# retab-dev/k-LLMs

Measured on NVIDIA H100. Metric: consensus records/sec at n=16 (1M x 32-field); achieved HBM GB/s vs peak, higher is better.
Workload: dtype i32 codes / f64 values

## Files before the change

### k_llms_b200/csrc/kc_jsongpu.cu

```cuda
#include <cuda_runtime.h>

#include <algorithm>
#include <atomic>
#include <chrono>
#include <cstdio>
#include <cstdlib>
#include <cstring>
#include <mutex>
#include <string>
#include <thread>
#include <type_traits>
#include <vector>

#include <cub/device/device_scan.cuh>
#include <nvtx3/nvToolsExt.h>

#include "../../include/kllms_b200.h"
#include "kc_internal.h"
#include "kc_jsongpu.cuh"

namespace {

using kc::js::Chunk;
using kc::js::Tok;
// ... 57 lines not shown
    }
    template <typename T>
    T *as() const { return static_cast<T *>(p); }
};

enum Stage { RECORDS, SLOTS, UNION, SCRATCH, CSR, OFF };
struct Units {
    size_t R, B, T = 0, P = 0, S = 0;
};
template <class Alloc>
int chunk_arrays(const Alloc &alloc, Chunk &ch, Stage stage, const Units &u, size_t keep, bool vrec) {
    const size_t n = (size_t)ch.n;
    int k = 0;
    auto a = [&](Stage st, auto *&ptr, size_t count, size_t per, size_t plus, int fill, bool on_device) {
        const int i = k++;
        return st == stage ? alloc(i, ptr, count * per + plus, keep * per, fill, on_device) : KC_OK;
    };
    R_(a(RECORDS, ch.fcount, u.R, 1, 1, 0, true));
    R_(a(RECORDS, ch.slot, u.R, 1, 1, 0, false));
    R_(a(RECORDS, ch.status, u.R, 1, 0, 0, false));
    R_(a(RECORDS, ch.nest, u.R, 1, 0, 0, false));
    R_(a(RECORDS, ch.pend, u.R, 1, 0, 0, false));
    R_(a(RECORDS, ch.plist, u.R, 1, 1, 0xFF, false));
    R_(a(ch.lists ? RECORDS : OFF, ch.lst, u.R, 1, 0, 0, false));
    R_(a(RECORDS, ch.vbase, u.R, 1, 0, 0, false));
    R_(a(RECORDS, ch.xbase, u.R, 1, 0, 0, false));
    R_(a(RECORDS, ch.mcount, u.R, 1, 1, 0, true));
    R_(a(RECORDS, ch.scount, u.R, 1, 1, 0, true));
    R_(a(RECORDS, ch.ccount, u.R, 1, 1, 0, true));
    R_(a(RECORDS, ch.len_c, u.R, 1, 1, 0, true));
    R_(a(RECORDS, ch.len_l, u.R, 1, 1, 0, true));
    R_(a(SLOTS, ch.toks, u.T, n, 1, 0, false));
    R_(a(SLOTS, ch.fdesc, u.T, 1, 1, 0, false));
    R_(a(SLOTS, ch.gpos, u.T, 1, 1, 0, false));
    R_(a(SLOTS, ch.piece_c, u.T, 1, 1, 0, false));
    R_(a(SLOTS, ch.piece_l, u.T, 1, 1, 0, false));
    R_(a(SLOTS, ch.vcells, u.T, n, 16, 0xFF, true));
    R_(a(SLOTS, ch.xcells, u.T, n, 2, 0, true));
    R_(a(vrec ? SLOTS : OFF, ch.vrec, u.T, 1, 1, 0xFF, false));
    R_(a(UNION, ch.ucand, u.P, n, 0, 0, false));
    R_(a(UNION, ch.ubase, u.P, 1, 0, 0, false));
    R_(a(UNION, ch.usize, u.P, 1, 0, 0, false));
    R_(a(SCRATCH, ch.utok, u.S, 1, 0, 0, false));
    R_(a(SCRATCH, ch.unode, u.S, 1, 0, 0, false));
    R_(a(SCRATCH, ch.umap, u.S, 1, 0, 0xFF, false));
    R_(a(CSR, ch.mchars, u.B, 1, 16, 0, false));
    R_(a(CSR, ch.mstr_off, u.T, n, 2, 0, false));
    R_(a(CSR, ch.mgrp_off, u.T, 1, 2, 0, false));
    return KC_OK;
}

void set_flags(Chunk &ch, uint32_t flags, uint8_t lists, int32_t aligned0) {
    ch.xmedoid = (flags & KC_JSON_NUMERIC_MEDOID) != 0;
    ch.key_union = (flags & KC_JSON_KEY_UNION) != 0;
    ch.unicode = (flags & KC_JSON_UNICODE) != 0;
    ch.lists = lists;
    ch.aligned0 = aligned0;
}

struct Worker {
    int device = -1;
    cudaStream_t stream = nullptr;
    cudaEvent_t ev[7] = {};
    DBuf text, off, counters, win, vmeta, xvalue, xmeta, out_c, out_l, scan_tmp, midx, mavg, seq, vweight;
    std::vector<DBuf> arrays;
    PBuf h_small;
// ... 635 lines not shown
    if (!res) return;
    release_blob(res->blob);
    delete res;
}


struct kc_debug_jsongpu {
    std::vector<int64_t> off;
    std::vector<uint8_t> text;
    int32_t n = 0;
    int64_t R = 0;
    std::vector<std::vector<uint8_t>> arrays;
    unsigned long long counters[6] = {0, 0, 0, 0, 0, 0};
    std::vector<uint8_t> out_c, out_l;
    int64_t R_out = 0;
    std::vector<int64_t> src;
    std::vector<int64_t> spliced_c, spliced_l;
    std::vector<uint8_t> spliced_out_c, spliced_out_l;
    Chunk ch{};
};

int kc_debug_jsongpu_plan(const char *h_text, const int64_t *h_off, int64_t n_records, int32_t n, kc_debug_jsongpu **out) {
    return kc_debug_jsongpu_plan_flags(h_text, h_off, n_records, n, 0u, out);
}

namespace {

void plan_twin(kc_debug_jsongpu *h, const char *h_text, const int64_t *h_off, int64_t R, int32_t n, uint32_t flags, uint8_t lists, int32_t aligned0) {
    h->R = R;
    h->R_out = R;
    h->n = n;
    h->off.assign(h_off, h_off + R * n + 1);
    h->text.assign((const uint8_t *)h_text + h_off[0], (const uint8_t *)h_text + h_off[R * n]);
    Chunk &ch = h->ch;
    ch.text = h->text.data();
    ch.off = h->off.data();
    ch.R = (int32_t)R;
    ch.n = n;
    ch.counters = h->counters;
    set_flags(ch, flags, lists, aligned0);
    auto host = [&](int k, auto *&ptr, size_t len, size_t, int fill, bool) -> int {
        using E = std::remove_reference_t<decltype(*ptr)>;
        if (h->arrays.size() <= (size_t)k) h->arrays.resize((size_t)k + 1);
        h->arrays[(size_t)k].resize(len * sizeof(E), (uint8_t)fill);
        ptr = reinterpret_cast<E *>(h->arrays[(size_t)k].data());
        return KC_OK;
    };
    Units u{(size_t)R, h->text.size()};
    chunk_arrays(host, ch, RECORDS, u, 0, true);
    for (int32_t r = 0; r < R; ++r) kc::js::count_record(ch, r);
    for (int64_t r = 0; r < R; ++r) ch.slot[r + 1] = ch.slot[r] + ch.fcount[r];
    u.T = ch.slot[R];
    chunk_arrays(host, ch, SLOTS, u, 0, true);
    const kc::js::HostTeam team{team_size(n)};
    for (int32_t r = 0; r < R; ++r) kc::js::plan_step(ch, r, team);
    if ((u.P = h->counters[3])) {
        const int32_t P = (int32_t)u.P;
        chunk_arrays(host, ch, UNION, u, 0, true);
        ch.uslot = (uint32_t)u.T;
        for (int32_t p = 0; p < P; ++p) kc::js::union_count_step(ch, p, team);
        u.S = std::max<size_t>(h->counters[4], 1);
        chunk_arrays(host, ch, SCRATCH, u, 0, true);
        for (int32_t p = 0; p < P; ++p) kc::js::union_build_step(ch, p, team);
        const size_t keep = u.T;
        u.T += h->counters[5];
        chunk_arrays(host, ch, SLOTS, u, keep, true);
        for (int32_t p = 0; p < P; ++p) kc::js::union_plan_step(ch, p, team);
    }
    for (uint32_t *cnt : {ch.mcount, ch.scount, ch.ccount}) exclusive_scan(cnt, u.R + 1);
    chunk_arrays(host, ch, CSR, u, 0, true);
    for (int32_t r = 0; r < R; ++r) kc::js::medoid_step(ch, r, team);
}

}

int kc_debug_jsongpu_plan_flags(const char *h_text, const int64_t *h_off, int64_t n_records, int32_t n, uint32_t flags,
                                kc_debug_jsongpu **out) {
    if (!h_text || !h_off || !out || n < 2 || n > KC_MAX_CANDIDATES || n_records < 0) return KC_EINVAL;
    const int64_t R = n_records;
    kc_debug_jsongpu *h = new kc_debug_jsongpu;
    const bool lists = (flags & KC_JSON_LISTS) != 0;
// ... 48 lines not shown
int kc_debug_jsongpu_set_medoid(kc_debug_jsongpu *h, const int32_t *medoid_idx, const double *medoid_avg) {
    if (!h) return KC_EINVAL;
    h->ch.midx = medoid_idx;
    h->ch.mavg = medoid_avg;
    return KC_OK;
}

int kc_debug_jsongpu_set_numeric_medoid(kc_debug_jsongpu *h, const int32_t *best, const double *best_avg) {
    if (!h) return KC_EINVAL;
    h->ch.xbest = best;
    h->ch.xavg = best_avg;
    return KC_OK;
}

int kc_debug_jsongpu_inputs(const kc_debug_jsongpu *h, const int8_t **vote_cells, int64_t *n_vote_groups, const double **num_cells,
                            int64_t *n_num_groups, const uint8_t **status) {
    if (!h) return KC_EINVAL;
    if (vote_cells) *vote_cells = h->ch.vcells;
    if (n_vote_groups) *n_vote_groups = (int64_t)h->counters[0];
    if (num_cells) *num_cells = h->ch.xcells;
    if (n_num_groups) *n_num_groups = (int64_t)h->counters[1];
    if (status) *status = h->ch.status;
    return KC_OK;
}

int kc_debug_jsongpu_emit(kc_debug_jsongpu *h, const uint32_t *vote_meta, const double *num_value, const uint32_t *num_meta,
                          const char **content, const int64_t **content_off, const char **likelihoods, const int64_t **likelihoods_off) {
    return kc_debug_jsongpu_emit_weighted(h, vote_meta, nullptr, num_value, num_meta, content, content_off, likelihoods, likelihoods_off);
}

int kc_debug_jsongpu_group_records(const kc_debug_jsongpu *h, const int32_t **group_record) {
    if (!h) return KC_EINVAL;
    if (group_record) *group_record = h->ch.vrec;
    return KC_OK;
}

int kc_debug_jsongpu_emit_weighted(kc_debug_jsongpu *h, const uint32_t *vote_meta, const float *vote_weight, const double *num_value,
                                   const uint32_t *num_meta, const char **content, const int64_t **content_off, const char **likelihoods,
                                   const int64_t **likelihoods_off) {
    if (!h) return KC_EINVAL;
    Chunk &ch = h->ch;
    ch.vmeta = vote_meta;
    ch.vweight = vote_weight;
    ch.xvalue = num_value;
    ch.xmeta = num_meta;
    const int64_t R = h->R;
    const kc::js::HostTeam team{team_size(h->n)};
    for (int32_t r = 0; r < R; ++r) kc::js::len_step(ch, r, team);
    exclusive_scan(ch.len_c, (size_t)R + 1);
    exclusive_scan(ch.len_l, (size_t)R + 1);
    const int64_t ac = ch.len_c[R], al = ch.len_l[R];
    h->out_c.assign((size_t)std::max<int64_t>(ac, 1), 0);
    h->out_l.assign((size_t)std::max<int64_t>(al, 1), 0);
    ch.out_c = h->out_c.data();
    ch.out_l = h->out_l.data();
    for (int32_t r = 0; r < R; ++r) kc::js::write_step(ch, r, team);
    if (h->R_out < R) {
        const int64_t Ro = h->R_out;
        std::vector<int64_t> from((size_t)Ro);
        for (int64_t r = 0; r < Ro; ++r) from[(size_t)r] = r;
        for (int64_t i = 0; i < R - Ro; ++i) {
            from[(size_t)h->src[(size_t)i]] = Ro + i;
            ch.status[h->src[(size_t)i]] = ch.status[Ro + i];
        }
        auto splice = [&](const int64_t *o, const std::vector<uint8_t> &blob, std::vector<int64_t> &so, std::vector<uint8_t> &sb) {
            so.assign((size_t)Ro + 1, 0);
// ... 249 lines not shown
```

### k_llms_b200/csrc/kc_jsongpu.cuh

```cuda
#pragma once

#include "kc_jsoncore.cuh"

namespace kc {
namespace js {

constexpr int32_t kMaxFields = 1024;

constexpr uint8_t D_UNION = 0xFF;
constexpr uint8_t D_LIST = 0xFE;

struct UNode {
    uint32_t kstart;
    uint16_t klen;
    uint8_t depth;
    uint8_t obj;
    uint8_t scalar;
    int32_t parent, child, last, next;
    int32_t lastc;
    uint32_t row, close;
};

KC_HD inline uint32_t fdesc_pack(uint32_t kind, uint32_t last, uint32_t rank, uint32_t gidx) { return kind | (last << 4) | (rank << 5) | (gidx << 16); }
KC_HD inline uint32_t fdesc_kind(uint32_t d) { return d & 15u; }
KC_HD inline uint32_t fdesc_last(uint32_t d) { return (d >> 4) & 1u; }
KC_HD inline uint32_t fdesc_rank(uint32_t d) { return (d >> 5) & 0x7FFu; }
KC_HD inline uint32_t fdesc_gidx(uint32_t d) { return d >> 16; }

struct Chunk {
    const uint8_t *text;
    const int64_t *off;
    int32_t R, n;
    uint32_t *fcount;
    uint8_t *nest;
    uint32_t *gpos;
    uint32_t *slot;
    uint8_t *status;
    Tok *toks;
    uint32_t *fdesc;
    uint32_t *vbase, *xbase;
    unsigned long long *counters;
    int8_t *vcells;
    double *xcells;
    uint32_t *mcount, *scount, *ccount;
    uint8_t *mchars;
    int32_t *mstr_off, *mgrp_off;
    const int32_t *midx;
    const double *mavg;
    int32_t *vrec;
    const float *vweight;
    const uint32_t *vmeta;
    const double *xvalue;
    const uint32_t *xmeta;
    bool xmedoid;
    const int32_t *xbest;
    const double *xavg;
    uint32_t *piece_c, *piece_l;
    int64_t *len_c, *len_l;
    uint8_t *out_c, *out_l;
    uint8_t *pend;
    int32_t *plist;
    uint32_t *ucand;
    uint32_t *ubase;
    uint32_t *usize;
    Tok *utok;
    UNode *unode;
    int32_t *umap;
    uint32_t uslot;
    bool key_union;
    uint8_t *lst;
    uint8_t lists;
    int32_t aligned0;
// ... 48 lines not shown
            decline(ch, r, D_LIST);
        } else if (f == -D_TOO_MANY_FIELDS || (f >= 0 && f != F)) {
            differ(ch, r, D_KEYS_DIFFER);
        } else if (f < 0) {
            decline(ch, r, -f);
        }
    }
}

KC_HD inline void settle_listed(const Chunk &ch, int32_t r) {
    int32_t why = D_LIST;
    for (int32_t c = 0; c < ch.n && why == D_LIST; ++c) {
        int64_t b, len;
        const int64_t base0 = ch.off[0];
        b = ch.off[(int64_t)r * ch.n + c] - base0;
        len = ch.off[(int64_t)r * ch.n + c + 1] - base0 - b;
        int32_t f = -D_TOO_LONG;
        if (len < ((int64_t)1 << 31)) f = scan_object(ch.text + b, (uint32_t)len, 0, nullptr, 0, kMaxFields, nullptr, true, nullptr, ch.unicode);
        if (f < 0) why = -f;
    }
    decline(ch, r, why);
}

KC_HD inline void sibling_range(const Tok *rt, int32_t n, int32_t F, int32_t j, uint32_t d, bool flat, int32_t &lo, int32_t &hi) {
    lo = 0;
    hi = F;
    if (flat) return;
    lo = j;
    while (lo > 0 && tok_depth(rt[(int64_t)(lo - 1) * n]) >= d) --lo;
    hi = j + 1;
    while (hi < F && tok_depth(rt[(int64_t)hi * n]) >= d) ++hi;
}

KC_HD inline void type_phase(const Chunk &ch, int32_t r, int32_t lane, int32_t team) {
    if (load_status(ch, r)) return;
    const int32_t F = (int32_t)ch.fcount[r], n = ch.n;
    const bool flat = ch.nest[r] == 0;
    const Tok *rt = ch.toks + (int64_t)ch.slot[r] * n;
    for (int32_t j = lane; j < F; j += team) {
        const Tok *row = rt + (int64_t)j * n;
        const uint32_t k0 = row[0].kind, d = tok_depth(row[0]);
        int32_t ref = j;
        if (is_close(k0)) {
            for (int32_t c = 1; c < n; ++c)
                if (row[c].kind != k0 || tok_depth(row[c]) != d) {
                    differ(ch, r, D_KEYS_DIFFER);
                    return;
                }
            ref = j - 1;
            while (ref > 0 && tok_depth(rt[(int64_t)ref * n]) != d) --ref;
        }
        const uint8_t *key = ch.text + rt[(int64_t)ref * n].kstart;
        const uint32_t klen = rt[(int64_t)ref * n].klen;
        const uint8_t elem = rt[(int64_t)ref * n].flags & TOK_ELEM;
        if (!is_close(k0)) {
            for (int32_t c = 1; c < n; ++c) {
                if ((row[c].kind == K_OPEN) != (k0 == K_OPEN) || (row[c].kind == K_LOPEN) != (k0 == K_LOPEN) || is_close(row[c].kind)) {
                    differ(ch, r, D_NESTED);
                    return;
                }
                if (tok_depth(row[c]) != d || (row[c].flags & TOK_ELEM) != elem || row[c].klen != klen ||
                    key_compare(ch.text + row[c].kstart, klen, key, klen) != 0) {
                    differ(ch, r, D_KEYS_DIFFER);
                    return;
                }
            }
            if (!elem && (contains(key, klen, "reasoning___", 12) || contains(key, klen, "source___", 9) ||
                          (F == 1 && klen == 4 && key_compare(key, 4, (const uint8_t *)"text", 4) == 0))) {
                decline(ch, r, D_SPECIAL_KEY);
                return;
            }
        }
        int32_t lo, hi;
        sibling_range(rt, n, F, ref, d, flat, lo, hi);
        uint32_t rank = 0, after = 0;
        for (int32_t i = lo; i < hi; ++i) {
            const Tok &o = rt[(int64_t)i * n];
            if (i == ref || (!flat && (tok_depth(o) != d || is_close(o.kind)))) continue;
            if (elem) {
                rank += i < ref ? 1u : 0u;
                after += i > ref ? 1u : 0u;
                continue;
            }
            const int cmp = key_compare(ch.text + o.kstart, o.klen, key, klen);
            if (cmp == 0) {
                decline(ch, r, D_DUP_KEY);
                return;
            }
            rank += cmp < 0 ? 1u : 0u;
            after += cmp > 0 ? 1u : 0u;
        }
        const uint32_t last = after == 0 ? 1u : 0u;
        if (is_open(k0) || is_close(k0)) {
            const uint32_t kind = k0 == K_OPEN ? F_OPEN : (k0 == K_CLOSE ? F_CLOSE : (k0 == K_LOPEN ? F_LOPEN : F_LCLOSE));
            ch.fdesc[ch.slot[r] + j] = fdesc_pack(kind, last, rank, 0);
            continue;
        }
        int32_t first = -1;
        for (int32_t c = 0; c < n && first < 0; ++c)
            if (row[c].kind != K_NULL) first = c;
        uint32_t kind;
        if (first < 0) {
            kind = F_ALLNULL;
        } else if (row[first].kind == K_STR) {
            kind = F_VOTE_STR;
            bool uni = false;
            for (int32_t c = 0; c < n; ++c) {
                if (row[c].kind == K_NULL) continue;
                if (row[c].kind != K_STR) {
                    decline(ch, r, D_MIXED_TYPES);
                    return;
                }
                if (row[c].flags & TOK_MULTIWORD) kind = F_MEDOID;
                uni |= (row[c].flags & TOK_UNICODE) != 0;
            }
            if (kind == F_VOTE_STR && uni) {
                decline(ch, r, D_ESCAPE_OR_NON_ASCII);
                return;
            }
            if (kind == F_MEDOID) {
                uint32_t live = 0, chars = 0, long_raw = 0, long_norm = 0;
                bool fits = true;
                for (int32_t c = 0; c < n; ++c) {
// ... 144 lines not shown
    const uint32_t n_groups = ch.mcount[ch.R], n_strings = ch.scount[ch.R];
    for (int32_t j = lane; j < F; j += team) {
        const uint32_t d = ch.fdesc[ch.slot[r] + j];
        if (fdesc_kind(d) != F_MEDOID) continue;
        const Tok *row = rt + (int64_t)j * n;
        uint32_t live = 0;
        for (int32_t c = 0; c < n; ++c) live += row[c].kind != K_NULL ? 1u : 0u;
        if (live < 2) continue;
        const uint32_t g = g0 + fdesc_gidx(d);
        uint32_t s = ch.scount[r] + ch.piece_c[ch.slot[r] + j], at = ch.ccount[r] + ch.piece_l[ch.slot[r] + j];
        ch.mgrp_off[g] = (int32_t)s;
        for (int32_t c = 0; c < n; ++c) {
            if (row[c].kind == K_NULL) continue;
            ch.mstr_off[s++] = (int32_t)at;
            const uint8_t *v = ch.text + row[c].vstart;
            at += (row[c].flags & TOK_UNICODE) ? normalize_string(v, row[c].vlen, ch.mchars + at) : sanitized_copy(v, row[c].vlen, ch.mchars + at);
        }
        if (g + 1 == n_groups) {
            ch.mgrp_off[n_groups] = (int32_t)n_strings;
            ch.mstr_off[n_strings] = (int32_t)at;
        }
    }
}

KC_HD inline void encode_phase(const Chunk &ch, int32_t r, int32_t lane, int32_t team) {
    if (load_status(ch, r)) return;
    const int32_t F = (int32_t)ch.fcount[r], n = ch.n;
    const Tok *rt = ch.toks + (int64_t)ch.slot[r] * n;
    for (int32_t j = lane; j < F; j += team) {
        const Tok *row = rt + (int64_t)j * n;
        const uint32_t d = ch.fdesc[ch.slot[r] + j], kind = fdesc_kind(d), g = fdesc_gidx(d);
        if (kind == F_VOTE_STR) {
            int8_t *cells = ch.vcells + ((int64_t)ch.vbase[r] + g) * n;
            int32_t n_classes = 0;
            for (int32_t c = 0; c < n; ++c) {
                if (row[c].kind == K_NULL) {
                    cells[c] = (int8_t)KC_CODE_NONE;
                    continue;
                }
                int32_t code = -1;
                for (int32_t p = 0; p < c && code < 0; ++p)
                    if (row[p].kind != K_NULL && cells[p] >= 0 &&
                        sanitized_equal(ch.text + row[p].vstart, row[p].vlen, ch.text + row[c].vstart, row[c].vlen))
                        code = cells[p];
                cells[c] = (int8_t)(code >= 0 ? code : n_classes++);
            }
        } else if (kind == F_VOTE_BOOL) {
            int8_t *cells = ch.vcells + ((int64_t)ch.vbase[r] + g) * n;
            for (int32_t c = 0; c < n; ++c) cells[c] = row[c].kind == K_TRUE ? 1 : 0;
        } else if (kind == F_NUMERIC) {
            double *cells = ch.xcells + ((int64_t)ch.xbase[r] + g) * n;
            for (int32_t c = 0; c < n; ++c) {
                const Tok &t = row[c];
                double v;
                if (t.kind == K_NULL) {
                    v = bits_f64(KC_F64_NONE_BITS);
                } else if (t.kind == K_INT || t.kind == K_FLOAT) {
                    if (!to_double(ch.text + t.vstart, t.vlen, v)) {
                        decline(ch, r, D_NUMBER_RANGE);
                        return;
                    }
                    if (t.kind == K_INT && v == 0.0) v = 0.0;
                } else {
                    v = bits_f64(0x7FF8000000000000ull);
                }
                cells[c] = v;
            }
        }
    }
}


KC_HD inline bool candidate_span(const Chunk &ch, int32_t r, int32_t c, int64_t &b, int64_t &len) {
    const int64_t base0 = ch.off[0];
    b = ch.off[(int64_t)r * ch.n + c] - base0;
    len = ch.off[(int64_t)r * ch.n + c + 1] - base0 - b;
    return len < ((int64_t)1 << 31) && b + len < ((int64_t)1 << 32);
}
// ... 347 lines not shown
#endif
    }
    template <class F>
    KC_HD void each(const F &f) const {
        if (live) f(lane);
        sync();
    }
    template <class F>
    KC_HD void leader(const F &f) const {
        if (live && lane == 0) f();
        sync();
    }
    template <class F>
    KC_HD void each_nosync(const F &f) const {
        if (live) f(lane);
    }
};

struct HostTeam {
    int32_t size;
    static constexpr bool live = true;
    template <class F>
    KC_HD void each(const F &f) const {
        for (int32_t lane = 0; lane < size; ++lane) f(lane);
    }
    template <class F>
    KC_HD void leader(const F &f) const { f(); }
    template <class F>
    KC_HD void each_nosync(const F &f) const { each(f); }
};

template <class Team>
KC_HD void table_phases(const Chunk &ch, int32_t r, const Team &tm, bool first_round) {
    tm.each([&](int32_t lane) { type_phase(ch, r, lane, tm.size); });
    tm.each([&](int32_t lane) { order_phase(ch, r, lane, tm.size); });
    tm.leader([&] { slots_phase(ch, r, first_round); });
    tm.each([&](int32_t lane) { encode_phase(ch, r, lane, tm.size); });
}

template <class Team>
KC_HD void plan_step(const Chunk &ch, int32_t r, const Team &tm) {
    tm.each([&](int32_t lane) { parse_phase(ch, r, lane, tm.size); });
    table_phases(ch, r, tm, true);
}

template <class Team>
KC_HD void union_count_step(const Chunk &ch, int32_t p, const Team &tm) {
    tm.each([&](int32_t lane) { union_count_phase(ch, p, lane, tm.size); });
    tm.leader([&] { union_reserve(ch, p); });
}

template <class Team>
KC_HD void union_build_step(const Chunk &ch, int32_t p, const Team &tm) {
    tm.each([&](int32_t lane) { union_scan_phase(ch, p, lane, tm.size); });
    tm.leader([&] { union_build(ch, p); });
}

template <class Team>
KC_HD void union_plan_step(const Chunk &ch, int32_t p, const Team &tm) {
    const int32_t r = tm.live ? ch.plist[p] : 0;
    tm.each([&](int32_t lane) { union_write_phase(ch, p, lane, tm.size); });
    tm.leader([&] {
        if (load_status(ch, r) == D_UNION) decline(ch, r, D_OK);
    });
    table_phases(ch, r, tm, false);
}
// ... 69 lines not shown
```

### include/kllms_b200.h

```cpp
#ifndef KLLMS_B200_H
#define KLLMS_B200_H

#include <stdint.h>

#ifdef __cplusplus
extern "C" {
#endif

#define KC_VERSION 200
#define KC_MAX_CANDIDATES 64

#define KC_OK 0
#define KC_EINVAL (-1)
#define KC_ECUDA (-2)
#define KC_ENODEV (-3)
#define KC_ENOMEM (-4)

#define KC_CODE_NONE (-1)
#define KC_CODE_ABSENT (-2)

#define KC_F64_NONE_BITS 0x7FF8C0DE00000000ULL
#define KC_F64_ABSENT_BITS 0x7FF8C0DF00000000ULL

#define KC_META_IDX(m) ((uint32_t)(m) & 0x3Fu)
// ... 116 lines not shown
void kc_free_strings(char **arr, int64_t count);

#define KC_JSON_DEVICE_ONLY 1u
#define KC_JSON_NUMERIC_MEDOID 2u
#define KC_JSON_KEY_UNION 4u
#define KC_JSON_LISTS 8u
#define KC_JSON_UNICODE 16u
typedef struct kc_json_result kc_json_result;
typedef struct {
    int64_t n_records, n_device, n_host, n_python;
    int64_t input_bytes, output_bytes;
    int32_t chunks, streams;
    double h2d_ms, plan_ms , kernel_ms , emit_ms , d2h_ms;
    double device_path_wall_ms, host_path_wall_ms, wall_ms;
} kc_json_stats;
int kc_consolidate_json_packed(const char *h_text, const int64_t *h_off, int64_t n_records, int32_t n, double rel_eps, double abs_eps,
                               int device, int32_t threads, uint32_t flags, kc_json_result **out);
int kc_consolidate_json_packed_weighted(const char *h_text, const int64_t *h_off, const float *h_seq_logprob, int64_t n_records, int32_t n,
                                        double rel_eps, double abs_eps, int device, int32_t threads, uint32_t flags, kc_json_result **out);
int kc_json_result_view(kc_json_result *res, const char **text, const int64_t **content_off, const int64_t **content_len,
                        const int64_t **likelihoods_off, const int64_t **likelihoods_len, const uint8_t **status, const uint8_t **why,
                        kc_json_stats *stats);
void kc_json_result_free(kc_json_result *res);

typedef struct kc_debug_jsongpu kc_debug_jsongpu;
int kc_debug_jsongpu_plan(const char *h_text, const int64_t *h_off, int64_t n_records, int32_t n, kc_debug_jsongpu **out);
int kc_debug_jsongpu_plan_flags(const char *h_text, const int64_t *h_off, int64_t n_records, int32_t n, uint32_t flags,
                                kc_debug_jsongpu **out);
int kc_debug_jsongpu_inputs(const kc_debug_jsongpu *h, const int8_t **vote_cells, int64_t *n_vote_groups, const double **num_cells,
                            int64_t *n_num_groups, const uint8_t **status);
int kc_debug_jsongpu_emit(kc_debug_jsongpu *h, const uint32_t *vote_meta, const double *num_value, const uint32_t *num_meta,
                          const char **content, const int64_t **content_off, const char **likelihoods, const int64_t **likelihoods_off);
int kc_debug_jsongpu_group_records(const kc_debug_jsongpu *h, const int32_t **group_record);
int kc_debug_jsongpu_emit_weighted(kc_debug_jsongpu *h, const uint32_t *vote_meta, const float *vote_weight, const double *num_value,
                                   const uint32_t *num_meta, const char **content, const int64_t **content_off, const char **likelihoods,
                                   const int64_t **likelihoods_off);
int kc_debug_jsongpu_medoid_inputs(const kc_debug_jsongpu *h, const uint8_t **chars, const int32_t **str_off, const int32_t **grp_off,
                                   int64_t *n_groups);
int kc_debug_jsongpu_set_medoid(kc_debug_jsongpu *h, const int32_t *medoid_idx, const double *medoid_avg);
int kc_debug_jsongpu_set_numeric_medoid(kc_debug_jsongpu *h, const int32_t *best, const double *best_avg);
void kc_debug_jsongpu_free(kc_debug_jsongpu *h);
int kc_debug_parse_doubles(const char *text, const int64_t *off, int64_t count, double *out, uint8_t *ok);
int kc_debug_float_reprs(const double *xs, int64_t count, char *out , int32_t *lens);
int kc_debug_parse_doubles_device(const char *text, const int64_t *off, int64_t count, double *out, uint8_t *ok, int device);
int kc_debug_float_reprs_device(const double *xs, int64_t count, char *out , int32_t *lens, int device);
int kc_debug_round5(const double *xs, int64_t count, double *out);
int kc_debug_s32_texts(uint64_t seed, int64_t n_records, int32_t n, int32_t threads, char *out, int64_t cap, int64_t *off);

int32_t kc_levenshtein(const char *a, int32_t alen, const char *b, int32_t blen);

void *kc_host_alloc(uint64_t bytes);
void kc_host_free(void *p);

#ifdef __cplusplus
}
#endif
#endif
```

### k_llms_b200/_native.py

```python
from __future__ import annotations

import ctypes
import os
from typing import Optional, Tuple

_HERE = os.path.dirname(os.path.abspath(__file__))
LIB_PATH = os.environ.get("KLLMS_B200_LIB") or os.path.join(_HERE, "libkllms_b200.so")

KC_OK, KC_EINVAL, KC_ECUDA, KC_ENODEV, KC_ENOMEM = 0, -1, -2, -3, -4
MAX_CANDIDATES = 64
CODE_NONE, CODE_ABSENT = -1, -2
F64_NONE_BITS = 0x7FF8C0DE00000000
F64_ABSENT_BITS = 0x7FF8C0DF00000000
FLAG_HAS_VALUE, FLAG_SINGLE, FLAG_TIE, FLAG_NO_FINITE = 1, 2, 4, 8
OUT_LOCAL, OUT_MULTIMEM, OUT_PEERS = 0, 1, 2

_vp, _i32, _i64, _u32, _u64, _f64 = ctypes.c_void_p, ctypes.c_int32, ctypes.c_int64, ctypes.c_uint32, ctypes.c_uint64, ctypes.c_double
_int, _str, _pp = ctypes.c_int, ctypes.c_char_p, ctypes.POINTER(ctypes.c_void_p)
_CONSENSUS_HOST = [_vp, _i32, _vp, _vp, _i32, _i64, _i32, _f64, _f64, _vp, _vp, _vp, _vp, _int, _vp]

_SIGNATURES = {
    "kc_version": (_int, []),
    "kc_last_error": (_str, []),
    "kc_device_count": (_int, []),
# ... 13 lines not shown
    "kc_logprob_sum_f32": (_int, [_vp, _vp, _i64, _vp, _vp]),
    "kc_weighted_vote_i32": (_int, [_vp, _vp, _i64, _i32, _i32, _vp, _vp, _vp, _vp, _vp]),
    "kc_weighted_vote_groups_i8": (_int, [_vp, _i64, _i32, _vp, _vp, _i64, _vp, _vp, _vp, _vp]),
    "kc_consensus_host": (_int, _CONSENSUS_HOST),
    "kc_consensus_host_i8": (_int, _CONSENSUS_HOST),
    "kc_host_alloc": (_vp, [_u64]),
    "kc_host_free": (None, [_vp]),
    "kc_medoid_str": (_int, [_vp, _vp, _vp, _i64, _i32, _vp, _vp, _vp]),
    "kc_medoid_str_method": (_int, [_vp, _vp, _vp, _i64, _i32, _i32, _vp, _vp, _vp]),
    "kc_medoid_str_host": (_int, [_vp, _i64, _vp, _vp, _i64, _i32, _vp, _vp, _int]),
    "kc_numeric_medoid_f64": (_int, [_vp, _i64, _i32, _vp, _vp, _vp]),
    "kc_levenshtein": (_int, [_str, _i32, _str, _i32]),
    "kc_consolidate_json": (_int, [_vp, _vp, _i64, _i32, _f64, _f64, _int, _i32, _vp, _vp, _vp]),
    "kc_free_strings": (None, [_vp, _i64]),
    "kc_align_json": (_int, [ctypes.POINTER(_str), _vp, _i32, _f64, ctypes.POINTER(_str)]),
    "kc_align_json_batch": (_int, [_vp, _vp, _i64, _i32, _f64, _int, _i32, _vp, _vp, _vp]),
    "kc_json_plan": (_int, [_vp, _vp, _i64, _i32, _i32, _pp]),
    "kc_json_inputs": (_int, [_vp] * 10),
    "kc_json_emit": (_int, [_vp] * 9),
    "kc_json_free": (None, [_vp]),
    "kc_consolidate_json_packed": (_int, [_vp, _vp, _i64, _i32, _f64, _f64, _int, _i32, _u32, _pp]),
    "kc_consolidate_json_packed_weighted": (_int, [_vp, _vp, _vp, _i64, _i32, _f64, _f64, _int, _i32, _u32, _pp]),
    "kc_json_result_view": (_int, [_vp] + [_pp] * 7 + [_vp]),
    "kc_json_result_free": (None, [_vp]),
    "kc_debug_similarity_json": (_int, [_str, _str, ctypes.POINTER(_f64)]),
    "kc_debug_lsap": (_int, [_i32, _i32, _vp, _vp, _vp]),
    "kc_debug_alignsim": (_int, [_vp, _i32, _vp]),
    "kc_debug_alignsim_nodes": (_int, [_vp, _vp, _i32, _i32, _int, _vp]),
    "kc_debug_jsongpu_plan": (_int, [_vp, _vp, _i64, _i32, _pp]),
    "kc_debug_jsongpu_plan_flags": (_int, [_vp, _vp, _i64, _i32, _u32, _pp]),
    "kc_debug_jsongpu_inputs": (_int, [_vp] * 6),
    "kc_debug_jsongpu_emit": (_int, [_vp, _vp, _vp, _vp] + [_pp] * 4),
    "kc_debug_jsongpu_group_records": (_int, [_vp, _pp]),
    "kc_debug_jsongpu_emit_weighted": (_int, [_vp, _vp, _vp, _vp, _vp] + [_pp] * 4),
    "kc_debug_jsongpu_medoid_inputs": (_int, [_vp] + [_pp] * 3 + [ctypes.POINTER(_i64)]),
    "kc_debug_jsongpu_set_medoid": (_int, [_vp, _vp, _vp]),
    "kc_debug_jsongpu_set_numeric_medoid": (_int, [_vp, _vp, _vp]),
    "kc_debug_jsongpu_free": (None, [_vp]),
    "kc_debug_parse_doubles": (_int, [_vp, _vp, _i64, _vp, _vp]),
    "kc_debug_float_reprs": (_int, [_vp, _i64, _vp, _vp]),
    "kc_debug_parse_doubles_device": (_int, [_vp, _vp, _i64, _vp, _vp, _int]),
    "kc_debug_float_reprs_device": (_int, [_vp, _i64, _vp, _vp, _int]),
    "kc_debug_round5": (_int, [_vp, _i64, _vp]),
    "kc_debug_s32_texts": (_int, [_u64, _i64, _i32, _i32, _vp, _i64, _vp]),
}
EXPORTS = tuple(_SIGNATURES)


class NativeError(RuntimeError):
    def __init__(self, code: int, what: str):
        super().__init__(f"libkllms_b200: {what} (code {code})")
        self.code = code


_lib: Optional[ctypes.CDLL] = None


def load() -> ctypes.CDLL:
    global _lib
    if _lib is not None:
        return _lib
    if not os.path.exists(LIB_PATH):
        raise ImportError(
            f"{LIB_PATH} not found: build the sm_90a library first (make -C k_llms_b200/csrc, or "
            "__graft_entry__.build()).  k_llms_b200 has no CPU fallback for the consensus hot path.")
    lib = ctypes.CDLL(LIB_PATH)
# ... 409 lines not shown
```

### k_llms_b200/csrc/kc_jsoncore.cuh

```cuda
#pragma once

#include <stdint.h>
#include <string.h>

#include "kc_internal.h"
#include "kc_ryu_tables.cuh"

namespace kc {
namespace js {

typedef unsigned __int128 u128;

enum : uint8_t { K_NULL = 0, K_TRUE = 1, K_FALSE = 2, K_INT = 3, K_FLOAT = 4, K_STR = 5, K_OPEN = 6, K_CLOSE = 7, K_LOPEN = 8, K_LCLOSE = 9 };
KC_HD inline bool is_open(uint32_t k) { return k == K_OPEN || k == K_LOPEN; }
KC_HD inline bool is_close(uint32_t k) { return k == K_CLOSE || k == K_LCLOSE; }
enum : uint8_t { F_ALLNULL = 0, F_VOTE_STR = 1, F_VOTE_BOOL = 2, F_NUMERIC = 3, F_MEDOID = 4, F_OPEN = 5, F_CLOSE = 6, F_LOPEN = 7, F_LCLOSE = 8 };
constexpr int32_t kMaxNesting = 8;

struct alignas(16) Tok {
    uint32_t vstart, vlen;
    uint32_t kstart;
    uint16_t klen;
    uint8_t kind;
    uint8_t flags;
// ... 290 lines not shown
    }
    while (p < len && is_json_ws(s[p])) ++p;
    if (p != len) return -D_SYNTAX;
    return j;
}


KC_HD inline bool is_alnum_lower(uint8_t &c) {
    if (c >= 'A' && c <= 'Z') c = (uint8_t)(c + 32);
    return (c >= 'a' && c <= 'z') || (c >= '0' && c <= '9');
}

KC_HD inline bool sanitized_equal(const uint8_t *a, uint32_t la, const uint8_t *b, uint32_t lb) {
    uint32_t i = 0, j = 0;
    for (;;) {
        uint8_t ca = 0, cb = 0;
        while (i < la) {
            ca = a[i];
            if (is_alnum_lower(ca)) break;
            i += ca == '\\' ? 2u : 1u;
        }
        while (j < lb) {
            cb = b[j];
            if (is_alnum_lower(cb)) break;
            j += cb == '\\' ? 2u : 1u;
        }
        if (i >= la || j >= lb) return i >= la && j >= lb;
        if (ca != cb) return false;
        ++i;
        ++j;
    }
}

KC_HD inline uint32_t sanitized_copy(const uint8_t *a, uint32_t la, uint8_t *out) {
    uint32_t k = 0;
    for (uint32_t i = 0; i < la; ++i) {
        uint8_t c = a[i];
        if (!is_alnum_lower(c)) {
            i += c == '\\' ? 1u : 0u;
            continue;
        }
        if (out) out[k] = c;
        ++k;
    }
    return k;
}

KC_HD inline uint32_t unescaped_length(const uint8_t *a, uint32_t la) {
    uint32_t k = 0;
    for (uint32_t i = 0; i < la; ++i, ++k) i += a[i] == '\\' ? 1u : 0u;
    return k;
}

KC_HD inline uint32_t decode_cp(const uint8_t *a, uint32_t la, uint32_t &i) {
    const uint8_t b = a[i];
    if (b == '\\') {
        const uint8_t e = a[i + 1];
        if (e != 'u') {
            i += 2;
            return e == 'b' ? 8u : (e == 'f' ? 12u : (e == 'n' ? 10u : (e == 'r' ? 13u : (e == 't' ? 9u : (uint32_t)e))));
        }
        uint32_t v, w;
        hex4(a + i + 2, v);
        i += 6;
        if (v >= 0xD800 && v < 0xDC00 && i + 6 <= la && a[i] == '\\' && a[i + 1] == 'u' && hex4(a + i + 2, w) && w >= 0xDC00 && w < 0xE000) {
            i += 6;
// ... 399 lines not shown
```

Baseline: 1.015 billion.

## Compare keys via packed 8-byte words and fast-path sorted sibling ranking

Keys are loaded as big-endian 64-bit words so equality and ordering checks mostly compare one integer instead of running a byte-wise compare. Sibling ranking first checks whether siblings are already sorted; if they are, rank comes straight from position, which replaces the per-field quadratic compare loop. For flat records the sortedness check runs once per lane rather than once per field. The text buffer is padded by 16 bytes so the unaligned word reads stay in bounds, and the device path relies on aligned 8-byte loads from the text buffer.

```diff
diff --git a/k_llms_b200/csrc/kc_jsongpu.cu b/k_llms_b200/csrc/kc_jsongpu.cu
--- a/k_llms_b200/csrc/kc_jsongpu.cu
+++ b/k_llms_b200/csrc/kc_jsongpu.cu
@@ -814,6 +814,8 @@
     h->n = n;
     h->off.assign(h_off, h_off + R * n + 1);
     h->text.assign((const uint8_t *)h_text + h_off[0], (const uint8_t *)h_text + h_off[R * n]);
+    const size_t bytes = h->text.size();
+    h->text.resize(bytes + 16, 0);
     Chunk &ch = h->ch;
     ch.text = h->text.data();
     ch.off = h->off.data();
@@ -828,7 +830,7 @@
         ptr = reinterpret_cast<E *>(h->arrays[(size_t)k].data());
         return KC_OK;
     };
-    Units u{(size_t)R, h->text.size()};
+    Units u{(size_t)R, bytes};
     chunk_arrays(host, ch, RECORDS, u, 0, true);
     for (int32_t r = 0; r < R; ++r) kc::js::count_record(ch, r);
     for (int64_t r = 0; r < R; ++r) ch.slot[r + 1] = ch.slot[r] + ch.fcount[r];
diff --git a/k_llms_b200/csrc/kc_jsongpu.cuh b/k_llms_b200/csrc/kc_jsongpu.cuh
--- a/k_llms_b200/csrc/kc_jsongpu.cuh
+++ b/k_llms_b200/csrc/kc_jsongpu.cuh
@@ -1,4 +1,6 @@
 #pragma once
+
+#include <cstring>
 
 #include "kc_jsoncore.cuh"
 
@@ -152,11 +154,63 @@
     while (hi < F && tok_depth(rt[(int64_t)hi * n]) >= d) ++hi;
 }
 
+KC_HD inline uint64_t bswap64(uint64_t x) {
+    x = ((x & 0x00FF00FF00FF00FFull) << 8) | ((x >> 8) & 0x00FF00FF00FF00FFull);
+    x = ((x & 0x0000FFFF0000FFFFull) << 16) | ((x >> 16) & 0x0000FFFF0000FFFFull);
+    return (x << 32) | (x >> 32);
+}
+
+KC_HD inline uint64_t text_word(const uint8_t *text, uint32_t a) {
+#ifdef __CUDA_ARCH__
+    return *(const uint64_t *)(text + a);
+#else
+    uint64_t w;
+    memcpy(&w, text + a, 8);
+    return w;
+#endif
+}
+
+KC_HD inline uint64_t key_word(const uint8_t *text, uint32_t kstart, uint32_t klen) {
+    if (klen == 0) return 0;
+    const uint32_t a = kstart & ~7u, sh = (kstart & 7u) * 8u;
+    uint64_t w = text_word(text, a) >> sh;
+    if (sh) w |= text_word(text, a + 8) << (64u - sh);
+    if (klen < 8) w &= (1ull << (8u * klen)) - 1ull;
+    return bswap64(w);
+}
+
+KC_HD inline uint64_t tok_word(const Chunk &ch, const Tok &t) { return key_word(ch.text, t.kstart, t.klen); }
+
+KC_HD inline int key_order(const Chunk &ch, uint64_t wa, const Tok &a, uint64_t wb, const Tok &b) {
+    if (wa != wb) return wa < wb ? -1 : 1;
+    if (a.klen <= 8 && b.klen <= 8) return 0;
+    return key_compare(ch.text + a.kstart + 8, a.klen - 8u, ch.text + b.kstart + 8, b.klen - 8u);
+}
+
+KC_HD inline bool sorted_rank(const Chunk &ch, const Tok *rt, int32_t n, int32_t lo, int32_t hi, int32_t ref, uint32_t d, bool flat,
+                              uint32_t &rank, uint32_t &after) {
+    rank = after = 0;
+    int32_t prev = -1;
+    uint64_t wprev = 0;
+    for (int32_t i = lo; i < hi; ++i) {
+        const Tok &t = rt[(int64_t)i * n];
+        if (!flat && (tok_depth(t) != d || is_close(t.kind))) continue;
+        const uint64_t w = tok_word(ch, t);
+        if (prev >= 0 && key_order(ch, wprev, rt[(int64_t)prev * n], w, t) >= 0) return false;
+        rank += i < ref ? 1u : 0u;
+        after += i > ref ? 1u : 0u;
+        prev = i;
+        wprev = w;
+    }
+    return true;
+}
+
 KC_HD inline void type_phase(const Chunk &ch, int32_t r, int32_t lane, int32_t team) {
     if (load_status(ch, r)) return;
     const int32_t F = (int32_t)ch.fcount[r], n = ch.n;
     const bool flat = ch.nest[r] == 0;
     const Tok *rt = ch.toks + (int64_t)ch.slot[r] * n;
+    int32_t flat_sorted = -1;
     for (int32_t j = lane; j < F; j += team) {
         const Tok *row = rt + (int64_t)j * n;
         const uint32_t k0 = row[0].kind, d = tok_depth(row[0]);
@@ -173,14 +227,15 @@
         const uint8_t *key = ch.text + rt[(int64_t)ref * n].kstart;
         const uint32_t klen = rt[(int64_t)ref * n].klen;
         const uint8_t elem = rt[(int64_t)ref * n].flags & TOK_ELEM;
+        const uint64_t wref = tok_word(ch, rt[(int64_t)ref * n]);
         if (!is_close(k0)) {
             for (int32_t c = 1; c < n; ++c) {
                 if ((row[c].kind == K_OPEN) != (k0 == K_OPEN) || (row[c].kind == K_LOPEN) != (k0 == K_LOPEN) || is_close(row[c].kind)) {
                     differ(ch, r, D_NESTED);
                     return;
                 }
-                if (tok_depth(row[c]) != d || (row[c].flags & TOK_ELEM) != elem || row[c].klen != klen ||
-                    key_compare(ch.text + row[c].kstart, klen, key, klen) != 0) {
+                if (tok_depth(row[c]) != d || (row[c].flags & TOK_ELEM) != elem || row[c].klen != klen || tok_word(ch, row[c]) != wref ||
+                    (klen > 8 && key_compare(ch.text + row[c].kstart + 8, klen - 8u, key + 8, klen - 8u) != 0)) {
                     differ(ch, r, D_KEYS_DIFFER);
                     return;
                 }
@@ -194,21 +249,34 @@
         int32_t lo, hi;
         sibling_range(rt, n, F, ref, d, flat, lo, hi);
         uint32_t rank = 0, after = 0;
-        for (int32_t i = lo; i < hi; ++i) {
-            const Tok &o = rt[(int64_t)i * n];
-            if (i == ref || (!flat && (tok_depth(o) != d || is_close(o.kind)))) continue;
-            if (elem) {
-                rank += i < ref ? 1u : 0u;
-                after += i > ref ? 1u : 0u;
-                continue;
-            }
-            const int cmp = key_compare(ch.text + o.kstart, o.klen, key, klen);
-            if (cmp == 0) {
-                decline(ch, r, D_DUP_KEY);
-                return;
-            }
-            rank += cmp < 0 ? 1u : 0u;
-            after += cmp > 0 ? 1u : 0u;
+        bool ranked = false;
+        if (flat) {
+            if (flat_sorted < 0) flat_sorted = sorted_rank(ch, rt, n, lo, hi, ref, d, true, rank, after) ? 1 : 0;
+            rank = (uint32_t)ref;
+            after = (uint32_t)(F - 1 - ref);
+            ranked = flat_sorted == 1;
+        } else if (!elem) {
+            ranked = sorted_rank(ch, rt, n, lo, hi, ref, d, false, rank, after);
+        }
+        if (!ranked) {
+            rank = after = 0;
+            const Tok &tref = rt[(int64_t)ref * n];
+            for (int32_t i = lo; i < hi; ++i) {
+                const Tok &o = rt[(int64_t)i * n];
+                if (i == ref || (!flat && (tok_depth(o) != d || is_close(o.kind)))) continue;
+                if (elem) {
+                    rank += i < ref ? 1u : 0u;
+                    after += i > ref ? 1u : 0u;
+                    continue;
+                }
+                const int cmp = key_order(ch, tok_word(ch, o), o, wref, tref);
+                if (cmp == 0) {
+                    decline(ch, r, D_DUP_KEY);
+                    return;
+                }
+                rank += cmp < 0 ? 1u : 0u;
+                after += cmp > 0 ? 1u : 0u;
+            }
         }
         const uint32_t last = after == 0 ? 1u : 0u;
         if (is_open(k0) || is_close(k0)) {
```

New measurement: 1.016 billion (median of 6 runs). No clear change (+0.2%).

## Precompute packed key and string prefix words to speed key ranking and vote encoding

Applied to the files above, without the earlier changes.

Adds a key_phase that packs the first 8 key bytes of each field into a big-endian 64-bit word, stored in a new per-slot kword buffer. The type phase then compares these words first and falls back to a full key_compare only on ties. Vote-string encoding now compares per-class sanitized 7-byte words with a length byte against class representatives instead of scanning every earlier candidate with sanitized_equal, and does the full comparison only for strings longer than 7 sanitized characters. This cuts text reads and byte-wise compares, at the cost of an extra phase, an extra buffer and per-thread local arrays of 64 words.

```diff
diff --git a/include/kllms_b200.h b/include/kllms_b200.h
--- a/include/kllms_b200.h
+++ b/include/kllms_b200.h
@@ -172,6 +172,8 @@
 int kc_debug_jsongpu_emit(kc_debug_jsongpu *h, const uint32_t *vote_meta, const double *num_value, const uint32_t *num_meta,
                           const char **content, const int64_t **content_off, const char **likelihoods, const int64_t **likelihoods_off);
 int kc_debug_jsongpu_group_records(const kc_debug_jsongpu *h, const int32_t **group_record);
+int kc_debug_jsongpu_table(const kc_debug_jsongpu *h, const uint32_t **fcount, const uint32_t **slot, const uint32_t **fdesc,
+                           const void **toks, const uint32_t **vbase, const uint8_t **text);
 int kc_debug_jsongpu_emit_weighted(kc_debug_jsongpu *h, const uint32_t *vote_meta, const float *vote_weight, const double *num_value,
                                    const uint32_t *num_meta, const char **content, const int64_t **content_off, const char **likelihoods,
                                    const int64_t **likelihoods_off);
diff --git a/k_llms_b200/_native.py b/k_llms_b200/_native.py
--- a/k_llms_b200/_native.py
+++ b/k_llms_b200/_native.py
@@ -69,6 +69,7 @@
     "kc_debug_jsongpu_inputs": (_int, [_vp] * 6),
     "kc_debug_jsongpu_emit": (_int, [_vp, _vp, _vp, _vp] + [_pp] * 4),
     "kc_debug_jsongpu_group_records": (_int, [_vp, _pp]),
+    "kc_debug_jsongpu_table": (_int, [_vp] + [_pp] * 6),
     "kc_debug_jsongpu_emit_weighted": (_int, [_vp, _vp, _vp, _vp, _vp] + [_pp] * 4),
     "kc_debug_jsongpu_medoid_inputs": (_int, [_vp] + [_pp] * 3 + [ctypes.POINTER(_i64)]),
     "kc_debug_jsongpu_set_medoid": (_int, [_vp, _vp, _vp]),
diff --git a/k_llms_b200/csrc/kc_jsoncore.cuh b/k_llms_b200/csrc/kc_jsoncore.cuh
--- a/k_llms_b200/csrc/kc_jsoncore.cuh
+++ b/k_llms_b200/csrc/kc_jsoncore.cuh
@@ -346,6 +346,27 @@
     }
 }
 
+KC_HD inline uint64_t sanitized_word(const uint8_t *a, uint32_t la) {
+    uint64_t w = 0;
+    uint32_t k = 0;
+    for (uint32_t i = 0; i < la; ++i) {
+        uint8_t c = a[i];
+        if (!is_alnum_lower(c)) {
+            i += c == '\\' ? 1u : 0u;
+            continue;
+        }
+        if (k < 7) w |= (uint64_t)c << (8 * k);
+        ++k;
+    }
+    return w | ((uint64_t)(k < 255u ? k : 255u) << 56);
+}
+
+KC_HD inline uint64_t key_word(const uint8_t *k, uint32_t kl) {
+    uint64_t w = 0;
+    for (uint32_t i = 0; i < 8; ++i) w = (w << 8) | (i < kl ? k[i] : 0u);
+    return w;
+}
+
 KC_HD inline uint32_t sanitized_copy(const uint8_t *a, uint32_t la, uint8_t *out) {
     uint32_t k = 0;
     for (uint32_t i = 0; i < la; ++i) {
diff --git a/k_llms_b200/csrc/kc_jsongpu.cu b/k_llms_b200/csrc/kc_jsongpu.cu
--- a/k_llms_b200/csrc/kc_jsongpu.cu
+++ b/k_llms_b200/csrc/kc_jsongpu.cu
@@ -113,6 +113,7 @@
     R_(a(RECORDS, ch.len_l, u.R, 1, 1, 0, true));
     R_(a(SLOTS, ch.toks, u.T, n, 1, 0, false));
     R_(a(SLOTS, ch.fdesc, u.T, 1, 1, 0, false));
+    R_(a(SLOTS, ch.kword, u.T, 1, 1, 0, false));
     R_(a(SLOTS, ch.gpos, u.T, 1, 1, 0, false));
     R_(a(SLOTS, ch.piece_c, u.T, 1, 1, 0, false));
     R_(a(SLOTS, ch.piece_l, u.T, 1, 1, 0, false));
@@ -943,6 +944,18 @@
 int kc_debug_jsongpu_group_records(const kc_debug_jsongpu *h, const int32_t **group_record) {
     if (!h) return KC_EINVAL;
     if (group_record) *group_record = h->ch.vrec;
+    return KC_OK;
+}
+
+int kc_debug_jsongpu_table(const kc_debug_jsongpu *h, const uint32_t **fcount, const uint32_t **slot, const uint32_t **fdesc,
+                           const void **toks, const uint32_t **vbase, const uint8_t **text) {
+    if (!h) return KC_EINVAL;
+    if (fcount) *fcount = h->ch.fcount;
+    if (slot) *slot = h->ch.slot;
+    if (fdesc) *fdesc = h->ch.fdesc;
+    if (toks) *toks = h->ch.toks;
+    if (vbase) *vbase = h->ch.vbase;
+    if (text) *text = h->ch.text;
     return KC_OK;
 }
 
diff --git a/k_llms_b200/csrc/kc_jsongpu.cuh b/k_llms_b200/csrc/kc_jsongpu.cuh
--- a/k_llms_b200/csrc/kc_jsongpu.cuh
+++ b/k_llms_b200/csrc/kc_jsongpu.cuh
@@ -38,6 +38,7 @@
     uint8_t *status;
     Tok *toks;
     uint32_t *fdesc;
+    uint64_t *kword;
     uint32_t *vbase, *xbase;
     unsigned long long *counters;
     int8_t *vcells;
@@ -152,11 +153,22 @@
     while (hi < F && tok_depth(rt[(int64_t)hi * n]) >= d) ++hi;
 }
 
+KC_HD inline void key_phase(const Chunk &ch, int32_t r, int32_t lane, int32_t team) {
+    if (load_status(ch, r)) return;
+    const int32_t F = (int32_t)ch.fcount[r], n = ch.n;
+    const Tok *rt = ch.toks + (int64_t)ch.slot[r] * n;
+    for (int32_t j = lane; j < F; j += team) {
+        const Tok &t = rt[(int64_t)j * n];
+        ch.kword[ch.slot[r] + j] = key_word(ch.text + t.kstart, t.klen);
+    }
+}
+
 KC_HD inline void type_phase(const Chunk &ch, int32_t r, int32_t lane, int32_t team) {
     if (load_status(ch, r)) return;
     const int32_t F = (int32_t)ch.fcount[r], n = ch.n;
     const bool flat = ch.nest[r] == 0;
     const Tok *rt = ch.toks + (int64_t)ch.slot[r] * n;
+    const uint64_t *kw = ch.kword + ch.slot[r];
     for (int32_t j = lane; j < F; j += team) {
         const Tok *row = rt + (int64_t)j * n;
         const uint32_t k0 = row[0].kind, d = tok_depth(row[0]);
@@ -194,15 +206,24 @@
         int32_t lo, hi;
         sibling_range(rt, n, F, ref, d, flat, lo, hi);
         uint32_t rank = 0, after = 0;
+        const uint64_t w = kw[ref];
         for (int32_t i = lo; i < hi; ++i) {
-            const Tok &o = rt[(int64_t)i * n];
-            if (i == ref || (!flat && (tok_depth(o) != d || is_close(o.kind)))) continue;
+            if (i == ref) continue;
+            if (!flat) {
+                const Tok &o = rt[(int64_t)i * n];
+                if (tok_depth(o) != d || is_close(o.kind)) continue;
+            }
             if (elem) {
                 rank += i < ref ? 1u : 0u;
                 after += i > ref ? 1u : 0u;
                 continue;
             }
-            const int cmp = key_compare(ch.text + o.kstart, o.klen, key, klen);
+            const uint64_t wi = kw[i];
+            int cmp = wi < w ? -1 : (wi > w ? 1 : 0);
+            if (cmp == 0) {
+                const Tok &o = rt[(int64_t)i * n];
+                cmp = key_compare(ch.text + o.kstart, o.klen, key, klen);
+            }
             if (cmp == 0) {
                 decline(ch, r, D_DUP_KEY);
                 return;
@@ -419,18 +440,26 @@
         const uint32_t d = ch.fdesc[ch.slot[r] + j], kind = fdesc_kind(d), g = fdesc_gidx(d);
         if (kind == F_VOTE_STR) {
             int8_t *cells = ch.vcells + ((int64_t)ch.vbase[r] + g) * n;
+            uint64_t word[KC_MAX_CANDIDATES];
+            uint8_t first[KC_MAX_CANDIDATES];
             int32_t n_classes = 0;
             for (int32_t c = 0; c < n; ++c) {
                 if (row[c].kind == K_NULL) {
                     cells[c] = (int8_t)KC_CODE_NONE;
                     continue;
                 }
+                const uint8_t *v = ch.text + row[c].vstart;
+                const uint64_t w = sanitized_word(v, row[c].vlen);
                 int32_t code = -1;
-                for (int32_t p = 0; p < c && code < 0; ++p)
-                    if (row[p].kind != K_NULL && cells[p] >= 0 &&
-                        sanitized_equal(ch.text + row[p].vstart, row[p].vlen, ch.text + row[c].vstart, row[c].vlen))
-                        code = cells[p];
-                cells[c] = (int8_t)(code >= 0 ? code : n_classes++);
+                for (int32_t k = 0; k < n_classes && code < 0; ++k)
+                    if (word[k] == w && ((w >> 56) <= 7u || sanitized_equal(ch.text + row[first[k]].vstart, row[first[k]].vlen, v, row[c].vlen)))
+                        code = k;
+                if (code < 0) {
+                    code = n_classes++;
+                    word[code] = w;
+                    first[code] = (uint8_t)c;
+                }
+                cells[c] = (int8_t)code;
             }
         } else if (kind == F_VOTE_BOOL) {
             int8_t *cells = ch.vcells + ((int64_t)ch.vbase[r] + g) * n;
@@ -844,6 +873,7 @@
 
 template <class Team>
 KC_HD void table_phases(const Chunk &ch, int32_t r, const Team &tm, bool first_round) {
+    tm.each([&](int32_t lane) { key_phase(ch, r, lane, tm.size); });
     tm.each([&](int32_t lane) { type_phase(ch, r, lane, tm.size); });
     tm.each([&](int32_t lane) { order_phase(ch, r, lane, tm.size); });
     tm.leader([&] { slots_phase(ch, r, first_round); });
```

Measured after the change: 1.004 billion before, 999.5 million after (median of 6 runs). Within noise of the previous version (-0.4%).
